# GUOShuxuan/kd-6d-pose-adlp

Measured on AMD Instinct MI355X. Metric: KD train-step images/sec (teacher+student fwd + OT loss + bwd + AdamW), higher is better.
Workload: dtype bf16

## Files before the change

### include/kd6d.h

```cpp
#ifndef KD6D_H
#define KD6D_H

#include <stdint.h>

#ifdef __cplusplus
extern "C" {
#endif

#define KD6D_ABI_VERSION 11

enum { KD6D_BF16 = 0, KD6D_F32 = 1 };
enum { KD6D_ACT_NONE = 0, KD6D_ACT_LEAKY = 1, KD6D_ACT_RELU = 2 };
enum {
  KD6D_OK = 0,
  KD6D_ERR_ARG = -1,
  KD6D_ERR_LAUNCH = -2,
  KD6D_ERR_UNSUPPORTED = -3
};

#define KD6D_MAX_SEG 5

typedef struct kd6d_seg {
  int32_t in_h, in_w;
  int32_t out_h, out_w;
// ... 60 lines not shown
  const kd6d_acc* sums;
  int32_t replicas;
  int32_t act;
  float eps;
  float momentum;
  const float* gamma;
  const float* beta;
  float* running_mean;
  float* running_var;
  float* save_mean;
  float* save_invstd;
} kd6d_bn_in;
int kd6d_conv2d_fwd_block(const kd6d_conv_geom* g, int dtype, const void* x, const kd6d_bn_in* bn, void* z_out,
                          const void* w, float* y_raw, kd6d_acc* stats, int stats_replicas, void* stream);

int kd6d_conv2d_dgrad(const kd6d_conv_geom* g, int dtype, const void* dy,
                      const void* wt, void* dx, int accumulate, void* stream);

int kd6d_conv2d_wgrad_parts(const kd6d_conv_geom* g, int dtype, int with_bias, int cu_budget);
int kd6d_conv2d_wgrad(const kd6d_conv_geom* g, int dtype, const void* x, const void* dy, float* dw_slab,
                      int64_t slab_floats, int64_t* dbias_acc, int64_t acc_hi_stride, int cu_budget, void* stream);

typedef struct kd6d_wgrad_item {
  kd6d_conv_geom geom;
  const void* x;
  const void* dy;
  float* dw;
  float* dbias;
} kd6d_wgrad_item;
int kd6d_wgrad_group_supported(const kd6d_conv_geom* g, int dtype);
int64_t kd6d_wgrad_group_plan(const kd6d_wgrad_item* items, int n_items, int dtype, int n_workgroups, void* plan_host,
                              int64_t plan_capacity, int32_t* info);
int kd6d_wgrad_group_launch(const void* plan_dev, int n_workgroups, int n_reduce_blocks, float* slab_dev, void* stream);

int kd6d_pack_dgrad_weights(int dtype, const void* w_base, void* wt_base,
                            const int32_t* desc_dev, int n_layers,
                            int total_blocks, void* stream);


typedef struct kd6d_levels {
  int32_t n;
  int32_t batch;
  int32_t h[KD6D_MAX_SEG];
  int32_t w[KD6D_MAX_SEG];
  float anchor_stride[KD6D_MAX_SEG];
  float anchor_size[KD6D_MAX_SEG];
} kd6d_levels;

#define KD6D_MAX_GT 4

int kd6d_device_cu_count(void);

typedef struct kd6d_ctx kd6d_ctx;
int kd6d_ctx_create(kd6d_ctx** out);
int kd6d_ctx_destroy(kd6d_ctx* ctx);
int kd6d_ctx_make_current(kd6d_ctx* ctx);
kd6d_ctx* kd6d_ctx_current(void);
int kd6d_ctx_set_option(kd6d_ctx* ctx, const char* name, long long value);
int kd6d_ctx_get_option(kd6d_ctx* ctx, const char* name, long long* value);
int kd6d_ctx_reset_options(kd6d_ctx* ctx);
int kd6d_ctx_barrier_timeouts(kd6d_ctx* ctx);
int kd6d_ctx_conv2d_pair_begin(kd6d_ctx* ctx);
int kd6d_ctx_conv2d_pair_end(kd6d_ctx* ctx);
int kd6d_ctx_conv2d_pair_pending(kd6d_ctx* ctx);

int kd6d_set_option(const char* name, long long value);
// ... 246 lines not shown
```

### kd-6d-pose-adlp_amd/build.py

```python
import hashlib
import os
import subprocess
import sys
from concurrent.futures import ThreadPoolExecutor

HERE = os.path.dirname(os.path.abspath(__file__))
CSRC = os.path.join(HERE, "csrc")
OUT = os.path.join(CSRC, "libkd6d.so")
HIPCC = os.environ.get("HIPCC", "/opt/rocm/bin/hipcc")
FLAGS = [
    "--offload-arch=gfx950", "-O3", "-fPIC", "-std=c++17", "-munsafe-fp-atomics",
    "-Wall", "-Wno-unused-function", "-Wno-unused-variable",
]


EXTRA_FLAGS = {"sinkhorn_dense.hip": ["-mllvm", "-amdgpu-mfma-vgpr-form"],
               "losses.hip": ["-Xclang", "-target-feature", "-Xclang", "-packed-fp32-ops"],
               "sinkhorn.hip": ["-Xclang", "-target-feature", "-Xclang", "-packed-fp32-ops"],
               "augment.hip": ["-Xclang", "-target-feature", "-Xclang", "-packed-fp32-ops"],
               "pnp.hip": ["-Xclang", "-target-feature", "-Xclang", "-packed-fp32-ops"],
               "pose_err.hip": ["-Xclang", "-target-feature", "-Xclang", "-packed-fp32-ops"],
               "bop_err.hip": ["-Xclang", "-target-feature", "-Xclang", "-packed-fp32-ops"],
               "bop_vsd.hip": ["-Xclang", "-target-feature", "-Xclang", "-packed-fp32-ops"],
               "render_frames.hip": ["-Xclang", "-target-feature", "-Xclang", "-packed-fp32-ops"]}


def _sources():
    return sorted(f for f in os.listdir(CSRC) if f.endswith(".hip"))


def _headers_digest():
    h = hashlib.sha256()
    for path in sorted([os.path.join(CSRC, n) for n in os.listdir(CSRC) if n.endswith(".h")]
                       + [os.path.join(HERE, "..", "include", "kd6d.h")]):
        with open(path, "rb") as f:
            h.update(os.path.basename(path).encode())
            h.update(f.read())
    h.update(" ".join(FLAGS).encode())
    return h


def _source_digest(src, base):
    h = base.copy()
    with open(os.path.join(CSRC, src), "rb") as f:
        h.update(f.read())
    h.update(" ".join(EXTRA_FLAGS.get(src, [])).encode())
    return h.hexdigest()


def _san_flags():
    import importlib.util
    path = os.path.join(HERE, "..", "tools", "build_sanitized.py")
    spec = importlib.util.spec_from_file_location("kd6d_build_sanitized", path)
    mod = importlib.util.module_from_spec(spec)
    spec.loader.exec_module(mod)
    return list(mod.SAN_FLAGS)

# ... 64 lines not shown
```

### kd-6d-pose-adlp_amd/csrc/kd6d_common.h

```cpp
#pragma once
#include <hip/hip_runtime.h>
#include <stdint.h>
#include <stdio.h>
#include <string.h>

#include "../../include/kd6d.h"

typedef __bf16 bf16_t;
typedef __bf16 bf16x8_t __attribute__((ext_vector_type(8)));
typedef __bf16 bf16x4_t __attribute__((ext_vector_type(4)));
typedef float f32x4_t __attribute__((ext_vector_type(4)));
typedef float f32x2_t __attribute__((ext_vector_type(2)));
typedef unsigned int u32x4_t __attribute__((ext_vector_type(4)));
typedef unsigned int u32x2_t __attribute__((ext_vector_type(2)));

void kd6d_set_error(const char* fmt, ...);

#define KD6D_CHECK_ARG(cond, ...)              \
  do {                                         \
    if (!(cond)) {                             \
      kd6d_set_error(__VA_ARGS__);             \
      return KD6D_ERR_ARG;                     \
    }                                          \
  } while (0)

#define KD6D_CHECK_LAUNCH(name)                                          \
  do {                                                                   \
    hipError_t e__ = hipGetLastError();                                  \
    if (e__ != hipSuccess) {                                             \
      kd6d_set_error("%s: launch failed: %s", name, hipGetErrorString(e__)); \
      return KD6D_ERR_LAUNCH;                                            \
    }                                                                    \
  } while (0)

enum Kd6dOption {
  KD6D_OPT_CONV_HALO = 0,
  KD6D_OPT_CONV_SMALLC,
  KD6D_OPT_CONV_SPLITK,
  KD6D_OPT_CONV_TILE,
  KD6D_OPT_WGRAD_SMALL,
  KD6D_OPT_BN_ONEPASS,
  KD6D_OPT_BN_ONEPASS_MAX,
  KD6D_OPT_GN_ONEPASS,
  KD6D_OPT_SINKHORN_LANES,
  KD6D_OPT_CONV_HALO_PAIRING,
  KD6D_OPT_CONV_FUSE_NORM,
  KD6D_OPT_SINKHORN_DENSE_MFMA,
  KD6D_OPT_CONV_HALO_WIDE,
  KD6D_OPT_CONV_SMALLC_WMAX,
  KD6D_OPT_SINKHORN_DENSE_SCREEN,
  KD6D_OPT_SINKHORN_DENSE_ROWS,
  KD6D_OPT_STEM_FUSED,
  KD6D_OPT_COUNT
};
long long kd6d_opt(int id);

struct kd6d_ctx {
  long long opt[KD6D_OPT_COUNT];
  void* pair;
  void (*pair_free)(void*);
  unsigned int* timeouts;
  bool owns_timeouts;
};
kd6d_ctx* kd6d_current_ctx();
unsigned int* kd6d_ctx_timeouts_ptr();

template <typename T> __device__ __forceinline__ float to_f32(T v);
template <> __device__ __forceinline__ float to_f32<float>(float v) { return v; }
template <> __device__ __forceinline__ float to_f32<bf16_t>(bf16_t v) { return (float)v; }

template <typename T> __device__ __forceinline__ T from_f32(float v);
template <> __device__ __forceinline__ float from_f32<float>(float v) { return v; }
template <> __device__ __forceinline__ bf16_t from_f32<bf16_t>(float v) { return (bf16_t)v; }

template <auto Kern>
static inline void kd6d_raise_lds_limit(size_t lds) {
  static size_t limit = 0;
  if (lds > limit) {
    (void)hipFuncSetAttribute(reinterpret_cast<const void*>(Kern), hipFuncAttributeMaxDynamicSharedMemorySize, (int)lds);
    limit = lds;
  }
}

template <typename T> struct Granule;
template <> struct Granule<bf16_t> { static constexpr int N = 8; };
// ... 54 lines not shown
```

### kd-6d-pose-adlp_amd/csrc/kd6d_core.hip

```cpp
#include <stdarg.h>

#include "kd6d_common.h"

namespace {
thread_local char g_err[512] = "";
}

void kd6d_set_error(const char* fmt, ...) {
  va_list ap;
  va_start(ap, fmt);
  vsnprintf(g_err, sizeof(g_err), fmt, ap);
  va_end(ap);
}

extern "C" const char* kd6d_last_error(void) { return g_err; }
extern "C" int kd6d_abi_version(void) { return KD6D_ABI_VERSION; }

namespace {
struct OptRow { const char* name; long long def; };
const OptRow kOptRows[KD6D_OPT_COUNT] = {
    {"conv.halo", -1},  {"conv.smallc", -1},       {"conv.splitk", -1}, {"conv.tile", -1},     {"wgrad.small", -1},
    {"bn.onepass", 1},  {"bn.onepass_max", 65536}, {"gn.onepass", 1},   {"sinkhorn.lanes", 1},
    {"conv.halo_pairing", 1}, {"conv.fuse_norm", 3}, {"sinkhorn.dense_mfma", 1}, {"conv.halo_wide", 1},
    {"conv.smallc_wmax", 640}, {"sinkhorn.dense_screen", 1}, {"sinkhorn.dense_rows", -1},
    {"stem.fused", 1},
};
int opt_index(const char* name) {
  if (!name) return -1;
  for (int i = 0; i < KD6D_OPT_COUNT; ++i)
    if (strcmp(name, kOptRows[i].name) == 0) return i;
  return -1;
}

void ctx_defaults(kd6d_ctx* c) {
  for (int i = 0; i < KD6D_OPT_COUNT; ++i) c->opt[i] = kOptRows[i].def;
  c->pair = nullptr; c->pair_free = nullptr; c->timeouts = nullptr; c->owns_timeouts = false;
}

kd6d_ctx* default_ctx() {
  static kd6d_ctx ctx = []() { kd6d_ctx c; ctx_defaults(&c); return c; }();
  return &ctx;
}
thread_local kd6d_ctx* g_current = nullptr;
}

namespace kd6d_detail { unsigned int* barrier_timeouts_device_ptr(); }

kd6d_ctx* kd6d_current_ctx() { return g_current ? g_current : default_ctx(); }

unsigned int* kd6d_ctx_timeouts_ptr() {
  kd6d_ctx* c = kd6d_current_ctx();
  if (!c->timeouts) c->timeouts = kd6d_detail::barrier_timeouts_device_ptr();
  return c->timeouts;
}

long long kd6d_opt(int id) { return kd6d_current_ctx()->opt[id]; }

extern "C" int kd6d_ctx_create(kd6d_ctx** out) {
// ... 168 lines not shown
```

### kd-6d-pose-adlp_amd/kd6d/_lib.py

```python
import ctypes
import os

_HERE = os.path.dirname(os.path.abspath(__file__))
LIB_PATH = os.path.join(os.path.dirname(_HERE), "csrc", "libkd6d.so")

KD6D_BF16 = 0
KD6D_F32 = 1
ACT_NONE, ACT_LEAKY, ACT_RELU = 0, 1, 2
GN_STATS_READY, GN_WS_ZEROED = 1, 2
MAX_SEG = 5
ABI_VERSION = 11
ACC_ACT, ACC_GRAD = 32, 52
NORM_GROUP, NORM_BATCH = 1, 2
BN_FUSED_REPLICAS = 8
NORM_MAX_CTILES = 8


class Seg(ctypes.Structure):
    _fields_ = [("in_h", ctypes.c_int32), ("in_w", ctypes.c_int32),
                ("out_h", ctypes.c_int32), ("out_w", ctypes.c_int32),
                ("in_row0", ctypes.c_int32), ("out_row0", ctypes.c_int32)]


class ConvGeom(ctypes.Structure):
# ... 54 lines not shown
SIGNATURES = {
    "kd6d_abi_version": [],
    "kd6d_device_cu_count": [],
    "kd6d_mark": [_P, _P],
    "kd6d_set_option": [ctypes.c_char_p, ctypes.c_longlong],
    "kd6d_get_option": [ctypes.c_char_p, ctypes.POINTER(ctypes.c_longlong)],
    "kd6d_reset_options": [],
    "kd6d_ctx_create": [ctypes.POINTER(_P)],
    "kd6d_ctx_destroy": [_P],
    "kd6d_ctx_current": [],
    "kd6d_ctx_make_current": [_P],
    "kd6d_ctx_set_option": [_P, ctypes.c_char_p, ctypes.c_longlong],
    "kd6d_ctx_get_option": [_P, ctypes.c_char_p, ctypes.POINTER(ctypes.c_longlong)],
    "kd6d_ctx_reset_options": [_P],
    "kd6d_ctx_barrier_timeouts": [_P],
    "kd6d_ctx_conv2d_pair_begin": [_P],
    "kd6d_ctx_conv2d_pair_end": [_P],
    "kd6d_ctx_conv2d_pair_pending": [_P],
    "kd6d_zero_regions": [ctypes.POINTER(ZeroList), _P, _I, _P],
    "kd6d_uniform_keys": [_P, _I64, _P, ctypes.c_uint64, _P],
    "kd6d_conv2d_fwd": [_G, _I, _P, _P, _P, _P, _P, _I, _P, _P, _I, _P, _I, _P, _I64, _P],
    "kd6d_conv2d_fwd_block": [_G, _I, _P, ctypes.POINTER(BnIn), _P, _P, _P, _P, _I, _P],
    "kd6d_conv2d_fwd_norm_fusable": [_G, _I, _I, _I],
    "kd6d_conv2d_fwd_norm": [_G, _I, _P, _P, _P, _P, ctypes.POINTER(ConvNorm), _P],
    "kd6d_conv2d_dgrad": [_G, _I, _P, _P, _P, _I, _P],
    "kd6d_conv2d_wgrad": [_G, _I, _P, _P, _P, _I64, _P, _I64, _I, _P],
    "kd6d_conv2d_wgrad_parts": [_G, _I, _I, _I],
    "kd6d_acc_read": [_P, _I64, _I, _P, _I, _I, _P],
    "kd6d_grad_acc_resolve": [_P, _I, _I, _P, _I64, _P, _P],
    "kd6d_grad_acc_resolve_part_groups": [_I],
    "kd6d_wgrad_group_supported": [_G, _I],
    "kd6d_wgrad_group_plan": [ctypes.POINTER(WgradItem), _I, _I, _I, _P, _I64, ctypes.POINTER(ctypes.c_int32)],
    "kd6d_wgrad_group_launch": [_P, _I, _I, _P, _P],
    "kd6d_pack_dgrad_weights": [_I, _P, _P, _P, _I, _I, _P],
    "kd6d_colstats": [_I, _P, _I64, _I, _P, _P, _P],
    "kd6d_bn_train_fwd": [_I, _I, _P, _P, _I64, _I, _P, _P, _P, _P, _F, _F, _P, _P, _P, _P, _I, _P],
    "kd6d_bn_train_fwd_res": [_I, _I, _P, _P, _P, _I64, _I, _P, _P, _P, _P, _F, _F, _P, _P, _P, _P, _I, _P],
    "kd6d_bn_train_bwd_reduce": [_I, _I, _P, _P, _I64, _I, _P, _P, _P, _P, _I, _P, _P, _I, _P],
    "kd6d_bn_train_bwd_apply": [_I, _I, _P, _P, _P, _I64, _I, _P, _P, _P, _P, _I, _P, _P, _P, _P, _I, _P],
    "kd6d_barrier_timeouts": [],
    "kd6d_conv2d_pair_begin": [],
    "kd6d_conv2d_pair_end": [],
    "kd6d_conv2d_pair_pending": [],
    "kd6d_bn_pool_train_fwd": [_I, _I, _P, _P, _I, _I, _I, _I, _P, _P, _P, _P, _F, _F, _P, _P, _P, _P, _I, _P],
    "kd6d_bn_pool_train_bwd": [_I, _I, _P, _P, _P, _I, _I, _I, _I, _P, _P, _P, _P, _I, _P, _P, _P, _P, _P, _I, _P],
    "kd6d_bn_pool_train_bwd_reduce": [_I, _I, _P, _P, _I, _I, _I, _I, _P, _P, _P, _P, _I, _P, _P, _I, _P],
    "kd6d_bn_pool_bwd_wgrad_parts": [_G, _I, _I],
    "kd6d_bn_pool_bwd_wgrad": [_G, _I, _P, _P, _P, _P, _P, _P, _P, _I, _P, _P, _I, _P, _P, _P, _I64, _I, _P],
    "kd6d_bn_train_bwd": [_I, _I, _P, _P, _P, _I64, _I, _P, _P, _P, _P, _I, _P, _P, _P, _P, _P, _I, _P],
    "kd6d_gn_relu_fwd": [_I, _I, _P, _P, ctypes.POINTER(ctypes.c_int32), _I, _I, _I, _I, _P, _P, _F, _P, _I, _P],
    "kd6d_gn_relu_bwd": [_I, _I, _P, _P, _P, ctypes.POINTER(ctypes.c_int32), _I, _I, _I, _I, _P, _P, _F, _P,
                         _P, _P, _P, _I64, _I, _P],
    "kd6d_gn_relu_bwd_pair": [_I, _I, ctypes.POINTER(GnItem), ctypes.POINTER(GnItem), ctypes.POINTER(ctypes.c_int32),
                              _I, _I, _I, _I, _F, _I64, _I, _P],
    "kd6d_maxpool2_fwd": [_I, _P, _P, _I, _I, _I, _I, _P],
    "kd6d_maxpool2_bwd": [_I, _P, _P, _P, _I, _I, _I, _I, _I, _P],
    "kd6d_upsample2_add": [_I, _P, _P, _P, _I, _I, _I, _I, _P],
    "kd6d_sumpool2": [_I, _P, _P, _I, _I, _I, _I, _I, _P],
    "kd6d_eltwise": [_I, _I, _P, _P, _P, _I64, _P],
    "kd6d_image_to_nhwc": [_I, _P, _P, _I, _I, _I, _I, _I, _P],
    "kd6d_sinkhorn_div_fwd_bwd": [_P, _P, _P, _P, _P, _P, _P, _P, _I, _F, _F, _F, _F, _P, _P, _P, _P, _P, _P],
    "kd6d_sinkhorn_max_points": [],
    "kd6d_sinkhorn_dense_workspace_floats": [_I, _I, _I],
    "kd6d_sinkhorn_dense_diameter": [_P, _P, _I, _I, _I, _P, _P, _P],
    "kd6d_sinkhorn_dense_fwd_bwd": [_P, _P, _P, _P, _I, _I, _I, _F, _F, _F, _F, _D, _P, _I64, _P, _P, _P, _P],
    "kd6d_teacher_select": [_L, _P, _P, _P, _F, _F, _F, _I, _F, _F, _P, _P, _P, _P, _P, _P, _P],
# ... 85 lines not shown
```

### kd-6d-pose-adlp_amd/kd6d/engine.py

```python
import math

import torch

from . import ops
from .ops import ACT_LEAKY, ACT_NONE, ACT_RELU

ANCHOR_SIZES = [32, 64, 128, 256, 512]
ANCHOR_STRIDES = [8, 16, 32, 64, 128]
TINY_CHANNELS = {
    "darknet_tiny": [[16], [32], [16, 128, 16, 128], [32, 256, 32, 256], [64, 512, 64, 512, 128]],
    "darknet_tiny_h": [[8], [16], [8, 64, 8, 64], [16, 128, 16, 128], [32, 256, 32, 256, 64]],
}
BACKBONE_CFG = {
    "darknet53": ([0, 0, 256, 512, 1024], 256),
    "darknet_tiny": ([0, 0, 128, 128], 256),
    "darknet_tiny_h": ([0, 0, 64, 64], 128),
}


def _pad8(c):
    return (c + 7) // 8 * 8


class Entry:
# ... 222 lines not shown
        return self.net.store.slab(self.w, parts)

    def stem_slab(self, g, dtype):
        budget = self.net.wgrad_budget()
        key = (id(g), dtype, "stem", budget, ops.get_option("stem.fused"))
        parts = self._parts.get(key)
        if parts is None:
            parts = self._parts[key] = ops.bn_pool_bwd_wgrad_parts(g, dtype, budget) if self.b is None else 0
        return self.net.store.slab(self.w, parts) if parts else None

    def bwd(self, x, dy, batch, levels, need_dx=True, dx=None, accumulate=False, need_dw=True):
        st = self.net.store
        g = self.geom(batch, levels)
        grp = self.net.wgrad_group if self.net.grouping else None
        if not need_dw:
            pass
        elif grp is not None and x.dtype == torch.bfloat16 and ops.wgrad_group_supported(g, x.dtype):
            grp.add(g, x, dy, st.storage(self.w, "grads"), None if self.b is None else st.storage(self.b, "grads"),
                    flops=self.flops(g))
        elif (side := self.net.next_side_stream()) is None:
            budget = self.net.wgrad_budget()
            ops.conv2d_wgrad(g, x, dy, self.wgrad_slab(g, x.dtype, budget), flops=self.flops(g),
                             dbias=None if self.b is None else st.acc(self.b), acc_stride=st.acc_stride, cu_budget=budget)
        else:
            budget = self.net.wgrad_budget()
            side.wait_stream(torch.cuda.current_stream())
            with torch.cuda.stream(side):
                ops.conv2d_wgrad(g, x, dy, self.wgrad_slab(g, x.dtype, budget), flops=self.flops(g),
                                 dbias=None if self.b is None else st.acc(self.b), acc_stride=st.acc_stride,
                                 cu_budget=budget)
        if not need_dx:
            return None
        return ops.conv2d_dgrad(g, dy, self.weight_t(), dx=dx, accumulate=accumulate, flops=self.flops(g))


class BatchNorm:
    def __init__(self, net, name, c, trainable=True):
        st = net.store
        self.net, self.c = net, c
        self.gamma = st.add(name + ".weight", "vec", (c,), (c,), trainable)
        self.beta = st.add(name + ".bias", "vec", (c,), (c,), trainable)
        self.rm = st.add(name + ".running_mean", "vec", (c,), (c,), False, region="buf")
        self.rv = st.add(name + ".running_var", "vec", (c,), (c,), False, region="buf")
        self.nbt_index = len(net.bns)
        net.bns.append((name, self))
        self.fold = None

    def folded(self):
        if self.fold is None:
            st = self.net.store
            scale = st.storage(self.gamma) * torch.rsqrt(st.storage(self.rv) + 1e-5)
            shift = st.storage(self.beta) - st.storage(self.rm) * scale
            self.fold = (scale.contiguous(), shift.contiguous())
        return self.fold


class ConvBlock:
    FUSE_STATS_MAX_ROWS = 1 << 15

    @staticmethod
    def bwd_replicas(rows):
        return 8 if rows >= (1 << 14) else 1

    def scratch_floats(self, rows):
        c, A, R = self.conv.cout_p, ops.ACC_FLOATS, self.bwd_replicas(rows)
        return (2 * A + 2 + 2 * A * R) * c + ops.BARRIER_WORDS
# ... 541 lines not shown
                        gn.fwd(raws[tname], B, levels_all, out=y)
                    saved[tname].append((xs[tname], raws[tname]))
                    xs[tname] = y
            for tname, tower, final in towers:
                seg = self.store.storage(self.scales) if tname == "pose" else None
                out, _ = final.fwd(xs[tname], B, levels_all, seg_scale=seg, out_f32=True,
                                   out=self.buf("%s.logits" % tname, (r, final.cout_p), torch.float32))
                self.head_ctx[tname] = (saved[tname], xs[tname])
                outs[tname] = out
            return outs["cls"], outs["pose"]
        for tname, tower, final in towers:
            x = head_in
            saved = []
            for li, (conv, gn) in enumerate(tower):
                y = self.buf("%s.act%d" % (tname, li), (r, oc))
                if self.fuse_norm_on() and conv.norm_fusable(B, levels_all, ops.NORM_GROUP, gn.groups):
                    raw = self.buf("%s.raw%d" % (tname, li), (r, oc), torch.float32) if self.training else None
                    gn.fwd_fused(conv, x, B, levels_all, y, raw_out=raw)
                else:
                    raw, _ = conv.fwd(x, B, levels_all, out_f32=True,
                                      out=self.buf("%s.raw%d" % (tname, li), (r, oc), torch.float32),
                                      stats=gn.stats(B, levels_all), stats_groups=gn.groups)
                    gn.fwd(raw, B, levels_all, out=y)
                saved.append((x, raw))
                x = y
                self._cut()
            seg = self.store.storage(self.scales) if tname == "pose" else None
            out, _ = final.fwd(x, B, levels_all, seg_scale=seg, out_f32=True,
                               out=self.buf("%s.logits" % tname, (r, final.cout_p), torch.float32))
            self.head_ctx[tname] = (saved, x)
            outs[tname] = out
        return outs["cls"], outs["pose"]

    def backward(self, dcls, dreg):
        assert self.training
        B, lv_all, r, oc = self.batch, self.levels, self.rows, self.out_channel
        if self.use_wgrad_group and self.dtype == torch.bfloat16 and self.wgrad_group is None:
            self.wgrad_group = ops.WgradGroup(self.wgrad_group_wgs or max(ops.device_cu_count() // 2, 1))
        self.grouping = self.wgrad_group is not None
        d_head_in = self.buf("d_head_in", (r, oc))
        first = True
        towers = (("cls", self.cls_tower, self.cls_logits, dcls), ("pose", self.pose_tower, self.pose_pred, dreg))
        if self.pair_towers:
            dxs = {}
            for tname, tower, final, dlog in towers:
                saved, last = self.head_ctx[tname]
                dxs[tname] = final.bwd(last, dlog, B, lv_all, dx=self.buf("%s.dact" % tname, (r, oc)))
            for li in range(len(self.cls_tower) - 1, -1, -1):
                draws, items = {}, []
                for tname, tower, _, _ in towers:
                    gn = tower[li][1]
                    draws[tname] = self.buf("%s.draw%d" % (tname, li), (r, oc))
                    items.append(gn.bwd_item(self.head_ctx[tname][0][li][1], dxs[tname], B, lv_all, draws[tname]))
                ops.gn_relu_bwd_pair(items, [h * w for (h, w) in lv_all], B, self.cls_tower[li][1].groups,
                                     self.store.acc_stride, flags=ops.GN_WS_ZEROED)
                if li > 0:
                    with ops.conv_pair(enabled=self.pair_towers == 1):
                        for tname, tower, _, _ in towers:
                            conv = tower[li][0]
                            dxs[tname] = conv.bwd(self.head_ctx[tname][0][li][0], draws[tname], B, lv_all,
                                                  dx=self.buf("%s.dact" % tname, (r, oc)))
                else:
                    for k, (tname, tower, _, _) in enumerate(towers):
                        tower[0][0].bwd(self.head_ctx[tname][0][0][0], draws[tname], B, lv_all, dx=d_head_in,
                                        accumulate=k > 0)
            towers = ()
        for tname, tower, final, dlog in towers:
            saved, last = self.head_ctx[tname]
            dx = final.bwd(last, dlog, B, lv_all, dx=self.buf("%s.dact" % tname, (r, oc)))
            for li in range(len(tower) - 1, -1, -1):
                conv, gn = tower[li]
                x_in, raw = saved[li]
                draw = gn.bwd(raw, dx, B, lv_all, self.buf("%s.draw%d" % (tname, li), (r, oc)))
                if li > 0:
                    dx = conv.bwd(x_in, draw, B, lv_all, dx=self.buf("%s.dact" % tname, (r, oc)))
                else:
                    conv.bwd(x_in, draw, B, lv_all, dx=d_head_in, accumulate=not first)
            first = False
        row0 = self.level_row0
        ops.mark("student.bwd.head.end")

        def dslot(li):
            h, w = lv_all[li]
            return d_head_in[row0[li]:row0[li] + B * h * w]

        idxs = sorted(self.inner.keys())
        n_l = len(idxs)
        grouped_out = set()
        if self.wgrad_group is not None:
            for pos in range(n_l):
                i = idxs[pos]
                f, lv, inner = self.fpn_ctx[i]
                conv = self.outc[i]
                g = conv.geom(B, lv)
                if ops.wgrad_group_supported(g, inner.dtype):
                    self.wgrad_group.add(g, inner, dslot(pos), self.store.storage(conv.w, "grads"),
                                         self.store.storage(conv.b, "grads"), flops=conv.flops(g))
                    grouped_out.add(i)
            if self.wgrad_group_flush != "fpn_end":
                self.flush_wgrad_group()
        self.grouping = False
        ftop, lvtop, p6, p6r, h6 = self.p6_ctx
# ... 83 lines not shown
```

### kd-6d-pose-adlp_amd/kd6d/models/model_kd.py

```python
import torch
from torch import nn

from .. import engine, kd_losses, ops
from ..kd_losses import KDLoss, PackedTargets, TeacherKnowledge


class _Shell(nn.Module):
    """Container used only to reproduce the reference's parameter hierarchy."""


def _get_shell(root, dotted):
    m = root
    for part in dotted:
        nxt = m._modules.get(part)
        if nxt is None:
            nxt = _Shell()
            m.add_module(part, nxt)
        m = nxt
    return m


class _StepFn(torch.autograd.Function):
    @staticmethod
    def forward(ctx, anchor, losses, module):
# ... 236 lines not shown
        tgt = targets if isinstance(targets, PackedTargets) else PackedTargets(targets, net.device)
        pre, side = None, net.side_stream
        keys = getattr(self, "_debug_keys", None)
        if side is not None and net.levels is not None and net.batch == B and net.in_hw == tuple(x.shape[-2:]):
            main = torch.cuda.current_stream()
            side.wait_stream(main)
            with torch.cuda.stream(side):
                pre = self.loss_evaluator.assign(net.levels, B, tgt, keys, prezeroed=prezeroed,
                                                 step_counter=self._nbt if prezeroed else None)
        cls, reg = net.forward(x, scratch_zeroed=prezeroed)
        if pre is not None:
            torch.cuda.current_stream().wait_stream(side)
        ops.mark("student.fwd.end")
        if isinstance(pred_t, kd_losses.DeferredTeacher):
            pred_t = pred_t.join()
        teacher = pred_t if isinstance(pred_t, TeacherKnowledge) else None
        if pred_t is not None and teacher is None:
            raise TypeError("pred_t must come from a kd6d teacher forward (TeacherKnowledge)")
        losses = self.loss_evaluator.forward(cls, reg, net.levels, B, tgt, teacher, keys=keys,
                                             seg_scale=st.storage(net.scales), pre=pre)
        ops.mark("student.loss.end")
        if not prezeroed:
            self._nbt += 1
        return losses

    def step_losses(self, images, targets, pred_t, weights):
        if not self.training:
            raise RuntimeError("step_losses() is the training step")
        x = images.tensors if hasattr(images, "tensors") else images
        if x.device != self.net.device:
            raise RuntimeError("images are on %s but the model is on %s" % (x.device, self.net.device))
        pre = self._begin_step(x)
        losses = self._forward_losses(x, targets, pred_t, prezeroed=pre)
        self._run_backward(weights, dreg_zeroed=pre)
        return losses

    def _run_backward(self, weights, dreg_zeroed=False):
        net, st = self.net, self.net.store
        first = _get_shell(self, ["head", "cls_logits"])._parameters["weight"]
        if first.grad is None:
            self._bind_grads()
        rows = net.rows
        dcls = net.buf("dcls", (rows, 16))
        dreg = net.buf("dreg", (rows, self.net.pose_pred.cout_p))
        if not dreg_zeroed:
            dreg.zero_()
        self.loss_evaluator.backward(weights, net.dtype, dcls, dreg, dseg_scale=st.acc(net.scales),
                                     acc_stride=st.acc_stride)
        ops.mark("student.bwd.start")
        from ..libs import distributed as D
        own = not getattr(self, "_defer_allreduce", False)
        split = D.bucket_split(st) if (own and D.exchange_active() and D.EXCHANGE_MODE == "overlap") else None
        if split is not None:
            comm = self._comm_stream = getattr(self, "_comm_stream", None) or torch.cuda.Stream()

            def early():
                for side in [torch.cuda.current_stream()] + list(net.side_streams or ([net.side_stream] if net.side_stream else [])):
                    comm.wait_stream(side)
                with torch.cuda.stream(comm):
                    st.resolve_grads(split, st.n_train)
                    D.exchange_slice(st, split, st.n_train)
            net.grad_hook = early
            net.resolve_hi = split
        try:
            net.backward(dcls, dreg)
        finally:
            if split is not None:
                net.grad_hook = None
                net.resolve_hi = None
        ops.mark("student.bwd.end")
        if split is not None:
            torch.cuda.current_stream().wait_stream(self._comm_stream)
            D.exchange_slice(st, 0, split)
        elif own:
            D.exchange_gradients(st)
```

### kd-6d-pose-adlp_amd/kd6d/ops.py

```python
import ctypes

import torch

from . import _lib
from ._lib import ACT_LEAKY, ACT_NONE, ACT_RELU, GN_STATS_READY, GN_WS_ZEROED, ConvGeom, check, lib


def dt_code(dtype):
    if dtype == torch.bfloat16:
        return _lib.KD6D_BF16
    if dtype == torch.float32:
        return _lib.KD6D_F32
    raise TypeError("kd6d supports bfloat16 and float32 activations, got %s" % dtype)


def granule(dtype):
    return 8 if dtype == torch.bfloat16 else 4


def _ptr(t):
    if t is None:
        return None
    assert t.is_cuda and t.is_contiguous(), "kd6d ops need contiguous device tensors"
    return ctypes.c_void_p(t.data_ptr())
# ... 164 lines not shown
    assert stats is None or (stats.dtype == torch.float32 and stats.numel() >= stats_replicas * 2 * geom.cout * ACC_FLOATS)
    bn = None
    if bn_in is not None:
        assert x.shape == (geom.rows_in, geom.cin) and x.dtype == torch.float32
        assert z_out is None or (z_out.shape == x.shape and z_out.dtype == w.dtype)
        bn = _lib.BnIn()
        bn.replicas, bn.act = int(bn_in["replicas"]), int(bn_in["act"])
        bn.eps, bn.momentum = float(bn_in.get("eps", 1e-5)), float(bn_in.get("momentum", 0.1))
        assert bn_in["sums"].numel() >= bn.replicas * 2 * geom.cin * ACC_FLOATS
        for name in ("sums", "gamma", "beta", "running_mean", "running_var", "save_mean", "save_invstd"):
            t = bn_in.get(name)
            assert t is None or (t.is_cuda and t.is_contiguous() and t.dtype == torch.float32)
            setattr(bn, name, t.data_ptr() if t is not None else None)
    else:
        assert x.shape == (geom.rows_in, geom.cin) and x.dtype == w.dtype and z_out is None
    with _Timed("conv_fwd", flops, geom):
        check(lib.kd6d_conv2d_fwd_block(geom.ref, dt_code(w.dtype), _ptr(x), ctypes.byref(bn) if bn is not None else None,
                                        _ptr(z_out), _ptr(w), _ptr(y_raw), _ptr(stats), int(stats_replicas), _stream()),
              "kd6d_conv2d_fwd_block")
    return y_raw


def conv2d_dgrad(geom, dy, wt, dx=None, accumulate=False, flops=0):
    assert dy.shape == (geom.rows_out, geom.cout), (dy.shape, geom.rows_out, geom.cout)
    assert wt.dtype == dy.dtype and wt.numel() == geom.cout * geom.ksize * geom.ksize * geom.cin
    if dx is None:
        assert not accumulate
        dx = torch.empty((geom.rows_in, geom.cin), dtype=dy.dtype, device=dy.device)
    assert dx.shape == (geom.rows_in, geom.cin) and dx.dtype == dy.dtype
    with _Timed("conv_dgrad", flops, geom):
        check(lib.kd6d_conv2d_dgrad(geom.ref, dt_code(dy.dtype), _ptr(dy), _ptr(wt), _ptr(dx),
                                    int(accumulate), _stream()), "kd6d_conv2d_dgrad")
    return dx


def conv2d_wgrad_parts(geom, dtype, with_bias=False, cu_budget=0):
    n = int(lib.kd6d_conv2d_wgrad_parts(geom.ref, dt_code(dtype), int(with_bias), int(cu_budget)))
    if n < 1:
        check(n, "kd6d_conv2d_wgrad_parts")
    return n


def conv2d_wgrad(geom, x, dy, dw_slab, flops=0, dbias=None, acc_stride=0, cu_budget=0):
    assert x.shape == (geom.rows_in, geom.cin) and dy.shape == (geom.rows_out, geom.cout)
    assert x.dtype == dy.dtype and dw_slab.dtype == torch.float32 and dw_slab.is_contiguous()
    assert dw_slab.numel() % (geom.cout * geom.ksize * geom.ksize * geom.cin) == 0
    with _Timed("conv_wgrad", flops, geom):
        assert dbias is None or (dbias.dtype == torch.int64 and dbias.numel() >= geom.cout and acc_stride > 0)
        check(lib.kd6d_conv2d_wgrad(geom.ref, dt_code(x.dtype), _ptr(x), _ptr(dy), _ptr(dw_slab), dw_slab.numel(),
                                    _ptr(dbias), int(acc_stride), int(cu_budget), _stream()), "kd6d_conv2d_wgrad")
    return dw_slab


def conv2d_wgrad_f32(geom, x, dy, with_bias=False, cu_budget=0):
    nw = geom.cout * geom.ksize * geom.ksize * geom.cin
    parts = conv2d_wgrad_parts(geom, x.dtype, with_bias, cu_budget)
    slab = torch.empty(parts, nw, dtype=torch.float32, device=x.device)
    acc = planar_acc(geom.cout, x.device) if with_bias else None
    conv2d_wgrad(geom, x, dy, slab, dbias=acc[:geom.cout] if with_bias else None, acc_stride=geom.cout,
                 cu_budget=cu_budget)
    dw = slab[0].clone()
    for k in range(1, parts):
        dw += slab[k]
    return dw, (planar_acc_value(acc) if with_bias else None)


# ... 739 lines not shown
```

Baseline: 6505.

## Add row-sparse backward for pose head conv using positive-anchor row lists

Result: no change. 6471 (-0.5%).

```diff
diff --git a/include/kd6d.h b/include/kd6d.h
--- a/include/kd6d.h
+++ b/include/kd6d.h
@@ -116,6 +116,12 @@
 int64_t kd6d_wgrad_group_plan(const kd6d_wgrad_item* items, int n_items, int dtype, int n_workgroups, void* plan_host,
                               int64_t plan_capacity, int32_t* info);
 int kd6d_wgrad_group_launch(const void* plan_dev, int n_workgroups, int n_reduce_blocks, float* slab_dev, void* stream);
+
+int kd6d_conv2d_rowsparse_supported(const kd6d_conv_geom* g, int dtype, int cap);
+int kd6d_conv2d_rowsparse_dgrad(const kd6d_conv_geom* g, int dtype, const void* dy, const void* wt, void* dx,
+                                int accumulate, const int32_t* cnt, const int32_t* row, int cap, void* stream);
+int kd6d_conv2d_rowsparse_wgrad(const kd6d_conv_geom* g, int dtype, const void* x, const void* dy, float* dw,
+                                float* dbias, const int32_t* cnt, const int32_t* row, int cap, void* stream);
 
 int kd6d_pack_dgrad_weights(int dtype, const void* w_base, void* wt_base,
                             const int32_t* desc_dev, int n_layers,
diff --git a/kd-6d-pose-adlp_amd/build.py b/kd-6d-pose-adlp_amd/build.py
--- a/kd-6d-pose-adlp_amd/build.py
+++ b/kd-6d-pose-adlp_amd/build.py
@@ -22,7 +22,8 @@
                "pose_err.hip": ["-Xclang", "-target-feature", "-Xclang", "-packed-fp32-ops"],
                "bop_err.hip": ["-Xclang", "-target-feature", "-Xclang", "-packed-fp32-ops"],
                "bop_vsd.hip": ["-Xclang", "-target-feature", "-Xclang", "-packed-fp32-ops"],
-               "render_frames.hip": ["-Xclang", "-target-feature", "-Xclang", "-packed-fp32-ops"]}
+               "render_frames.hip": ["-Xclang", "-target-feature", "-Xclang", "-packed-fp32-ops"],
+               "conv_rowsparse.hip": ["-Xclang", "-target-feature", "-Xclang", "-packed-fp32-ops"]}
 
 
 def _sources():
diff --git a/kd-6d-pose-adlp_amd/csrc/conv_rowsparse.hip b/kd-6d-pose-adlp_amd/csrc/conv_rowsparse.hip
--- /dev/null
+++ b/kd-6d-pose-adlp_amd/csrc/conv_rowsparse.hip
@@ -0,0 +1,391 @@
+#include "kd6d_common.h"
+
+namespace {
+
+struct RsLevels {
+  int n, batch, rows;
+  int h[KD6D_MAX_SEG], w[KD6D_MAX_SEG], row0[KD6D_MAX_SEG];
+};
+
+constexpr int kDgWaves = 4;
+constexpr int kDgTile = 64;
+constexpr int kWgThreads = 1024;
+constexpr int kWgWaves = kWgThreads / 64;
+constexpr int kWgSlotsPerThread = 4;
+constexpr int kWgMaxSlots = kWgThreads * kWgSlotsPerThread;
+constexpr int kWgBatch = 8;
+constexpr int kCoBlock = 16, kCiTile = 128, kMaxCout = 256;
+
+__device__ __forceinline__ float bf16_lo(unsigned v) { return __uint_as_float(v << 16); }
+__device__ __forceinline__ float bf16_hi(unsigned v) { return __uint_as_float(v & 0xffff0000u); }
+
+__device__ __forceinline__ int level_of(const RsLevels& L, int r) {
+  int l = 0;
+#pragma unroll
+  for (int s = 1; s < KD6D_MAX_SEG; ++s)
+    if (s < L.n && r >= L.row0[s]) l = s;
+  return l;
+}
+__device__ __forceinline__ void level_dims(const RsLevels& L, int l, int& h, int& w, int& row0) {
+  h = L.h[0]; w = L.w[0]; row0 = L.row0[0];
+#pragma unroll
+  for (int s = 1; s < KD6D_MAX_SEG; ++s)
+    if (s == l) { h = L.h[s]; w = L.w[s]; row0 = L.row0[s]; }
+}
+
+typedef __bf16 rs_bf16x8 __attribute__((ext_vector_type(8)));
+
+__global__ __launch_bounds__(kDgWaves * 64) void rowsparse_dgrad_kernel(
+    const RsLevels L, const bf16_t* __restrict__ dy, const bf16_t* __restrict__ wt, bf16_t* __restrict__ dx,
+    const int* __restrict__ cnt, const int* __restrict__ rowlist, int cap, int cin, int cout, int accumulate) {
+  const int lane = threadIdx.x & 63;
+  const int fr = lane & 15, fq = lane >> 4;
+  const int p = blockIdx.x * kDgWaves + __builtin_amdgcn_readfirstlane((int)(threadIdx.x >> 6));
+  if (p >= L.rows) return;
+  int h, w, row0;
+  level_dims(L, level_of(L, p), h, w, row0);
+  const int hw = h * w;
+  const int b = (p - row0) / hw;
+  const int img0 = row0 + b * hw;
+  const int py = (p - img0) / w, px = (p - img0) - py * w;
+  int tq[9];
+#pragma unroll
+  for (int t = 0; t < 9; ++t) tq[t] = -1;
+  bool any = false;
+  const int n = cnt[b];
+  for (int s0 = 0; s0 < cap; s0 += 64) {
+    const int s = s0 + lane;
+    int tap = -1, q = -1;
+    if (s < cap) q = rowlist[(size_t)b * cap + s];
+    if (s < n) {
+      const int c = q - img0;
+      if (c >= 0 && c < hw) {
+        const int qy = c / w, qx = c - qy * w;
+        const int ky = py - qy + 1, kx = px - qx + 1;
+        if (ky >= 0 && ky <= 2 && kx >= 0 && kx <= 2) tap = ky * 3 + kx;
+      }
+    }
+    if (__ballot(tap >= 0) == 0ull) continue;
+    any = true;
+#pragma unroll
+    for (int t = 0; t < 9; ++t) {
+      const unsigned long long m = __ballot(tap == t);
+      if (tq[t] < 0 && m) tq[t] = __builtin_amdgcn_readlane(q, __ffsll((long long)m) - 1);
+    }
+  }
+  if (!any) {
+    if (!accumulate)
+      for (int c = 8 * lane; c < cin; c += 512)
+        *reinterpret_cast<u32x4_t*>(dx + (size_t)p * cin + c) = u32x4_t{0u, 0u, 0u, 0u};
+    return;
+  }
+
+  u32x2_t dv[9];
+#pragma unroll
+  for (int t = 0; t < 9; ++t) {
+    dv[t] = u32x2_t{0u, 0u};
+    if (tq[t] >= 0 && 4 * lane < cout)
+      dv[t] = *reinterpret_cast<const u32x2_t*>(dy + (size_t)tq[t] * cout + 4 * lane);
+  }
+  unsigned bm[9];
+#pragma unroll
+  for (int t = 0; t < 9; ++t) {
+    unsigned long long m = __ballot(((dv[t].x | dv[t].y) & 0x7fff7fffu) != 0u);
+    m |= m >> 1; m |= m >> 2;
+    unsigned bits = 0u;
+#pragma unroll
+    for (int k = 0; k < kMaxCout / kCoBlock; ++k) bits |= (unsigned)((m >> (4 * k)) & 1ull) << k;
+    bm[t] = bits;
+  }
+
+  const int nb = cout / kCoBlock;
+  const int K = 9 * cout;
+  for (int c0 = 0; c0 < cin; c0 += kDgTile) {
+    f32x4_t acc[kDgTile / 16];
+#pragma unroll
+    for (int i = 0; i < kDgTile / 16; ++i) acc[i] = f32x4_t{0.f, 0.f, 0.f, 0.f};
+    int last_j = -1;
+#pragma unroll
+    for (int t = 0; t < 9; ++t) {
+      unsigned m = bm[t];
+      while (m) {
+        const int blk = __ffs((int)m) - 1;
+        m &= m - 1u;
+        const int j = (t * nb + blk) >> 1;
+        if (j == last_j) continue;
+        last_j = j;
+        const int kk = 32 * j + 8 * fq;
+        const int g = 2 * j + (fq >> 1);
+        int q = tq[t], tl = t;
+        if (t + 1 < 9 && g >= (t + 1) * nb) { q = tq[t + 1 < 9 ? t + 1 : t]; tl = t + 1; }
+        if (t > 0 && g < t * nb) { q = tq[t > 0 ? t - 1 : t]; tl = t - 1; }
+        const bool kvalid = kk < K;
+        rs_bf16x8 fb = {0, 0, 0, 0, 0, 0, 0, 0};
+        if (q >= 0 && kvalid)
+          fb = *reinterpret_cast<const rs_bf16x8*>(dy + (size_t)q * cout + (kk - tl * cout));
+        rs_bf16x8 fa[kDgTile / 16];
+#pragma unroll
+        for (int i = 0; i < kDgTile / 16; ++i) {
+          fa[i] = rs_bf16x8{0, 0, 0, 0, 0, 0, 0, 0};
+          if (kvalid) fa[i] = *reinterpret_cast<const rs_bf16x8*>(wt + (size_t)(c0 + 16 * i + fr) * K + kk);
+        }
+#pragma unroll
+        for (int i = 0; i < kDgTile / 16; ++i)
+          acc[i] = __builtin_amdgcn_mfma_f32_16x16x32_bf16(fa[i], fb, acc[i], 0, 0, 0);
+      }
+    }
+    if (fr < kDgTile / 16) {
+      f32x4_t v = acc[0];
+#pragma unroll
+      for (int i = 1; i < kDgTile / 16; ++i)
+        if (fr == i) v = acc[i];
+      u32x2_t* out = reinterpret_cast<u32x2_t*>(dx + (size_t)p * cin + c0 + 16 * fr + 4 * fq);
+      if (accumulate) {
+        const u32x2_t old = *out;
+        v[0] += bf16_lo(old.x); v[1] += bf16_hi(old.x); v[2] += bf16_lo(old.y); v[3] += bf16_hi(old.y);
+      }
+      *out = u32x2_t{pack_bf16x2(v[0], v[1]), pack_bf16x2(v[2], v[3])};
+    }
+  }
+}
+
+__global__ __launch_bounds__(kWgThreads) void rowsparse_wgrad_kernel(
+    const RsLevels L, const bf16_t* __restrict__ x, const bf16_t* __restrict__ dy, float* __restrict__ dw,
+    float* __restrict__ dbias, const int* __restrict__ cnt, const int* __restrict__ rowlist, int cap, int cin,
+    int cout) {
+  __shared__ __attribute__((aligned(16))) int s_buf[2 * kWgMaxSlots];
+  __shared__ int s_wcnt[kWgWaves];
+  __shared__ float s_bias[kWgWaves][kCoBlock];
+  int* s_q = s_buf;
+  int* s_n = s_buf + kWgMaxSlots;
+  const int tid = threadIdx.x, lane = tid & 63;
+  const int wave = __builtin_amdgcn_readfirstlane(tid >> 6);
+  const int cb = blockIdx.x, tap = blockIdx.y, c0 = blockIdx.z * kCiTile;
+  const int ky = tap / 3, kx = tap - ky * 3;
+  const int nslots = L.batch * cap;
+  const bool do_bias = dbias != nullptr && tap == 4 && blockIdx.z == 0;
+
+  int myr[kWgSlotsPerThread], myn[kWgSlotsPerThread];
+#pragma unroll
+  for (int k = 0; k < kWgSlotsPerThread; ++k) {
+    const int i = tid + k * kWgThreads;
+    int r = -1;
+    if (i < nslots) {
+      const int b = i / cap, s = i - b * cap;
+      if (s < cnt[b]) {
+        r = rowlist[i];
+        if (r < 0 || r >= L.rows) r = -1;
+      }
+    }
+    myr[k] = r;
+    s_q[i] = r;
+  }
+  __syncthreads();
+#pragma unroll
+  for (int k = 0; k < kWgSlotsPerThread; ++k) {
+    const int i = tid + k * kWgThreads;
+    int r = myr[k], nb = -1;
+    if (r >= 0) {
+      const int b = i / cap, s = i - b * cap;
+      int h, w, row0;
+      level_dims(L, level_of(L, r), h, w, row0);
+      const int hw = h * w;
+      const int c = r - row0 - b * hw;
+      bool keep = c >= 0 && c < hw;
+      for (int e = 0; keep && e < s; ++e) keep = s_q[b * cap + e] != r;
+      if (keep) {
+        const u32x4_t* d = reinterpret_cast<const u32x4_t*>(dy + (size_t)r * cout + cb * kCoBlock);
+        const u32x4_t d0 = d[0], d1 = d[1];
+        keep = (((d0.x | d0.y | d0.z | d0.w) | (d1.x | d1.y | d1.z | d1.w)) & 0x7fff7fffu) != 0u;
+      }
+      if (keep) {
+        const int y = c / w, xx = c - y * w;
+        const int ny = y + ky - 1, nx = xx + kx - 1;
+        keep = ny >= 0 && ny < h && nx >= 0 && nx < w;
+        nb = r + (ky - 1) * w + (kx - 1);
+      }
+      if (!keep) r = -1;
+    }
+    myr[k] = r; myn[k] = nb;
+  }
+  __syncthreads();
+  int n = 0;
+#pragma unroll
+  for (int k = 0; k < kWgSlotsPerThread; ++k) {
+    if (k * kWgThreads >= nslots) break;
+    const bool valid = myr[k] >= 0;
+    const unsigned long long m = __ballot(valid);
+    if (lane == 0) s_wcnt[wave] = __popcll(m);
+    __syncthreads();
+    int off = n, tot = 0;
+#pragma unroll
+    for (int v = 0; v < kWgWaves; ++v) {
+      const int c = s_wcnt[v];
+      if (v < wave) off += c;
+      tot += c;
+    }
+    if (valid) {
+      const int pos = off + __popcll(m & ((1ull << lane) - 1ull));
+      s_q[pos] = myr[k]; s_n[pos] = myn[k];
+    }
+    n += tot;
+    __syncthreads();
+  }
+  if (n == 0) return;
+
+  const int lo = (int)((long long)n * wave / kWgWaves), hi = (int)((long long)n * (wave + 1) / kWgWaves);
+  float acc[kCoBlock][2];
+#pragma unroll
+  for (int c = 0; c < kCoBlock; ++c) acc[c][0] = acc[c][1] = 0.f;
+  const bf16_t* xl = x + c0 + 2 * lane;
+  const bf16_t* dyb = dy + cb * kCoBlock;
+  for (int i = lo; i < hi; i += kWgBatch) {
+    unsigned xv[kWgBatch];
+    u32x4_t d0[kWgBatch], d1[kWgBatch];
+#pragma unroll
+    for (int j = 0; j < kWgBatch; ++j) {
+      xv[j] = 0u; d0[j] = d1[j] = u32x4_t{0u, 0u, 0u, 0u};
+      if (i + j < hi) {
+        const int q = __builtin_amdgcn_readfirstlane(s_q[i + j]);
+        const int nb = __builtin_amdgcn_readfirstlane(s_n[i + j]);
+        xv[j] = *reinterpret_cast<const unsigned*>(xl + (size_t)nb * cin);
+        const u32x4_t* d = reinterpret_cast<const u32x4_t*>(dyb + (size_t)q * cout);
+        d0[j] = d[0]; d1[j] = d[1];
+      }
+    }
+#pragma unroll
+    for (int j = 0; j < kWgBatch; ++j) {
+      if (i + j >= hi) break;
+      const float x0 = bf16_lo(xv[j]), x1 = bf16_hi(xv[j]);
+      const unsigned dd[8] = {d0[j].x, d0[j].y, d0[j].z, d0[j].w, d1[j].x, d1[j].y, d1[j].z, d1[j].w};
+#pragma unroll
+      for (int c = 0; c < 8; ++c) {
+        const float da = bf16_lo(dd[c]), db = bf16_hi(dd[c]);
+        acc[2 * c][0] = fmaf(da, x0, acc[2 * c][0]);
+        acc[2 * c][1] = fmaf(da, x1, acc[2 * c][1]);
+        acc[2 * c + 1][0] = fmaf(db, x0, acc[2 * c + 1][0]);
+        acc[2 * c + 1][1] = fmaf(db, x1, acc[2 * c + 1][1]);
+      }
+    }
+  }
+  if (do_bias) {
+    float bs = 0.f;
+    if (lane < kCoBlock) {
+#pragma unroll 8
+      for (int i = lo; i < hi; ++i) bs += to_f32<bf16_t>(dyb[(size_t)s_q[i] * cout + lane]);
+      s_bias[wave][lane] = bs;
+    }
+  }
+  __syncthreads();
+
+  float* s_part = reinterpret_cast<float*>(s_buf);
+  constexpr int kTile = kCoBlock * kCiTile;
+  float t0 = 0.f, t1 = 0.f;
+  for (int round = 0; round < kWgWaves / 4; ++round) {
+    if ((wave >> 2) == round) {
+      float* dst = s_part + (wave & 3) * kTile + 2 * lane;
+#pragma unroll
+      for (int c = 0; c < kCoBlock; ++c) *reinterpret_cast<f32x2_t*>(dst + c * kCiTile) = f32x2_t{acc[c][0], acc[c][1]};
+    }
+    __syncthreads();
+#pragma unroll
+    for (int v = 0; v < 4; ++v) {
+      const f32x2_t pv = *reinterpret_cast<const f32x2_t*>(s_part + v * kTile + 2 * tid);
+      t0 += pv.x; t1 += pv.y;
+    }
+    __syncthreads();
+  }
+  {
+    const int c = tid >> 6, ci = c0 + 2 * lane;
+    f32x2_t* out = reinterpret_cast<f32x2_t*>(dw + ((size_t)(cb * kCoBlock + c) * 9 + tap) * cin + ci);
+    f32x2_t o = *out;
+    o.x += t0; o.y += t1;
+    *out = o;
+  }
+  if (do_bias && tid < kCoBlock) {
+    float bs = 0.f;
+#pragma unroll
+    for (int v = 0; v < kWgWaves; ++v) bs += s_bias[v][tid];
+    dbias[cb * kCoBlock + tid] += bs;
+  }
+}
+
+int rowsparse_params(const kd6d_conv_geom* g, int dtype, int cap, const char* who, RsLevels& L, bool quiet) {
+  if (quiet) {
+    if (!g || dtype != KD6D_BF16 || g->nseg < 1 || g->nseg > KD6D_MAX_SEG || g->ksize != 3 || g->stride != 1 ||
+        g->pad != 1 || g->batch < 1 || cap < 1 || g->cin <= 0 || g->cin % kCiTile || g->cout <= 0 ||
+        g->cout % kCoBlock || g->cout > kMaxCout || (long long)g->batch * cap > kWgMaxSlots)
+      return KD6D_ERR_UNSUPPORTED;
+  } else {
+    KD6D_CHECK_ARG(g != nullptr, "%s: null geometry", who);
+    KD6D_CHECK_ARG(g->nseg >= 1 && g->nseg <= KD6D_MAX_SEG && g->batch >= 1 && cap >= 1, "%s: nseg=%d batch=%d cap=%d",
+                   who, g->nseg, g->batch, cap);
+    if (dtype != KD6D_BF16 || g->ksize != 3 || g->stride != 1 || g->pad != 1 || g->cin <= 0 || g->cin % kCiTile ||
+        g->cout <= 0 || g->cout % kCoBlock || g->cout > kMaxCout || (long long)g->batch * cap > kWgMaxSlots) {
+      kd6d_set_error("%s: takes bf16, 3x3 / stride 1 / pad 1, cin %% %d == 0, cout %% %d == 0, cout <= %d, batch * cap "
+                     "<= %d (got dtype %d, k %d, stride %d, pad %d, cin %d, cout %d, batch %d, cap %d)", who, kCiTile,
+                     kCoBlock, kMaxCout, kWgMaxSlots, dtype, g->ksize, g->stride, g->pad, g->cin, g->cout, g->batch, cap);
+      return KD6D_ERR_UNSUPPORTED;
+    }
+  }
+  long long rows = 0;
+  L.n = g->nseg; L.batch = g->batch;
+  for (int s = 0; s < KD6D_MAX_SEG; ++s) { L.h[s] = L.w[s] = 1; L.row0[s] = 0; }
+  for (int s = 0; s < g->nseg; ++s) {
+    const kd6d_seg& q = g->seg[s];
+    const bool ok = q.in_h > 0 && q.in_w > 0 && q.out_h == q.in_h && q.out_w == q.in_w && q.in_row0 == rows &&
+                    q.out_row0 == rows && (long long)q.in_h * q.in_w <= (1 << 24);
+    if (!ok) {
+      if (!quiet) kd6d_set_error("%s: level %d is not a packed stride-1 level (%dx%d -> %dx%d, rows %d / %d)", who, s,
+                                 q.in_h, q.in_w, q.out_h, q.out_w, q.in_row0, q.out_row0);
+      return quiet ? KD6D_ERR_UNSUPPORTED : KD6D_ERR_ARG;
+    }
+    L.h[s] = q.in_h; L.w[s] = q.in_w; L.row0[s] = (int)rows;
+    rows += (long long)g->batch * q.in_h * q.in_w;
+    if (rows >= (1ll << 30)) {
+      if (!quiet) kd6d_set_error("%s: grid too large", who);
+      return quiet ? KD6D_ERR_UNSUPPORTED : KD6D_ERR_ARG;
+    }
+  }
+  L.rows = (int)rows;
+  return KD6D_OK;
+}
+
+}
+
+extern "C" int kd6d_conv2d_rowsparse_supported(const kd6d_conv_geom* g, int dtype, int cap) {
+  const long long opt = kd6d_opt(KD6D_OPT_HEAD_ROWSPARSE_BWD);
+  if (opt == 0) return 0;
+  RsLevels L;
+  if (rowsparse_params(g, dtype, cap, "kd6d_conv2d_rowsparse_supported", L, true) != KD6D_OK) return 0;
+  return opt == 2 ? 2 : 1;
+}
+
+extern "C" int kd6d_conv2d_rowsparse_dgrad(const kd6d_conv_geom* g, int dtype, const void* dy, const void* wt, void* dx,
+                                           int accumulate, const int32_t* cnt, const int32_t* row, int cap,
+                                           void* stream) {
+  RsLevels L;
+  int rc = rowsparse_params(g, dtype, cap, "kd6d_conv2d_rowsparse_dgrad", L, false);
+  if (rc) return rc;
+  KD6D_CHECK_ARG(dy && wt && dx && cnt && row, "kd6d_conv2d_rowsparse_dgrad: null tensor pointer");
+  hipLaunchKernelGGL(rowsparse_dgrad_kernel, dim3((unsigned)cdiv(L.rows, kDgWaves)), dim3(kDgWaves * 64), 0,
+                     reinterpret_cast<hipStream_t>(stream), L, reinterpret_cast<const bf16_t*>(dy),
+                     reinterpret_cast<const bf16_t*>(wt), reinterpret_cast<bf16_t*>(dx), cnt, row, cap, g->cin, g->cout,
+                     accumulate ? 1 : 0);
+  KD6D_CHECK_LAUNCH("kd6d_conv2d_rowsparse_dgrad");
+  return KD6D_OK;
+}
+
+extern "C" int kd6d_conv2d_rowsparse_wgrad(const kd6d_conv_geom* g, int dtype, const void* x, const void* dy, float* dw,
+                                           float* dbias, const int32_t* cnt, const int32_t* row, int cap,
+                                           void* stream) {
+  RsLevels L;
+  int rc = rowsparse_params(g, dtype, cap, "kd6d_conv2d_rowsparse_wgrad", L, false);
+  if (rc) return rc;
+  KD6D_CHECK_ARG(x && dy && dw && cnt && row, "kd6d_conv2d_rowsparse_wgrad: null tensor pointer");
+  hipLaunchKernelGGL(rowsparse_wgrad_kernel, dim3((unsigned)(g->cout / kCoBlock), 9u, (unsigned)(g->cin / kCiTile)),
+                     dim3(kWgThreads), 0, reinterpret_cast<hipStream_t>(stream), L, reinterpret_cast<const bf16_t*>(x),
+                     reinterpret_cast<const bf16_t*>(dy), dw, dbias, cnt, row, cap, g->cin, g->cout);
+  KD6D_CHECK_LAUNCH("kd6d_conv2d_rowsparse_wgrad");
+  return KD6D_OK;
+}
diff --git a/kd-6d-pose-adlp_amd/csrc/kd6d_common.h b/kd-6d-pose-adlp_amd/csrc/kd6d_common.h
--- a/kd-6d-pose-adlp_amd/csrc/kd6d_common.h
+++ b/kd-6d-pose-adlp_amd/csrc/kd6d_common.h
@@ -51,6 +51,7 @@
   KD6D_OPT_SINKHORN_DENSE_SCREEN,
   KD6D_OPT_SINKHORN_DENSE_ROWS,
   KD6D_OPT_STEM_FUSED,
+  KD6D_OPT_HEAD_ROWSPARSE_BWD,
   KD6D_OPT_COUNT
 };
 long long kd6d_opt(int id);
diff --git a/kd-6d-pose-adlp_amd/csrc/kd6d_core.hip b/kd-6d-pose-adlp_amd/csrc/kd6d_core.hip
--- a/kd-6d-pose-adlp_amd/csrc/kd6d_core.hip
+++ b/kd-6d-pose-adlp_amd/csrc/kd6d_core.hip
@@ -23,7 +23,7 @@
     {"bn.onepass", 1},  {"bn.onepass_max", 65536}, {"gn.onepass", 1},   {"sinkhorn.lanes", 1},
     {"conv.halo_pairing", 1}, {"conv.fuse_norm", 3}, {"sinkhorn.dense_mfma", 1}, {"conv.halo_wide", 1},
     {"conv.smallc_wmax", 640}, {"sinkhorn.dense_screen", 1}, {"sinkhorn.dense_rows", -1},
-    {"stem.fused", 1},
+    {"stem.fused", 1},  {"head.rowsparse_bwd", 1},
 };
 int opt_index(const char* name) {
   if (!name) return -1;
diff --git a/kd-6d-pose-adlp_amd/kd6d/_lib.py b/kd-6d-pose-adlp_amd/kd6d/_lib.py
--- a/kd-6d-pose-adlp_amd/kd6d/_lib.py
+++ b/kd-6d-pose-adlp_amd/kd6d/_lib.py
@@ -110,6 +110,9 @@
     "kd6d_wgrad_group_supported": [_G, _I],
     "kd6d_wgrad_group_plan": [ctypes.POINTER(WgradItem), _I, _I, _I, _P, _I64, ctypes.POINTER(ctypes.c_int32)],
     "kd6d_wgrad_group_launch": [_P, _I, _I, _P, _P],
+    "kd6d_conv2d_rowsparse_supported": [_G, _I, _I],
+    "kd6d_conv2d_rowsparse_dgrad": [_G, _I, _P, _P, _P, _I, _P, _P, _I, _P],
+    "kd6d_conv2d_rowsparse_wgrad": [_G, _I, _P, _P, _P, _P, _P, _P, _I, _P],
     "kd6d_pack_dgrad_weights": [_I, _P, _P, _P, _I, _I, _P],
     "kd6d_colstats": [_I, _P, _I64, _I, _P, _P, _P],
     "kd6d_bn_train_fwd": [_I, _I, _P, _P, _I64, _I, _P, _P, _P, _P, _F, _F, _P, _P, _P, _P, _I, _P],
diff --git a/kd-6d-pose-adlp_amd/kd6d/engine.py b/kd-6d-pose-adlp_amd/kd6d/engine.py
--- a/kd-6d-pose-adlp_amd/kd6d/engine.py
+++ b/kd-6d-pose-adlp_amd/kd6d/engine.py
@@ -278,6 +278,24 @@
         if not need_dx:
             return None
         return ops.conv2d_dgrad(g, dy, self.weight_t(), dx=dx, accumulate=accumulate, flops=self.flops(g))
+
+    def rowsparse_mode(self, batch, levels, cap):
+        key = (batch, tuple(levels), cap, self.net.dtype, "rowsparse", ops.get_option("head.rowsparse_bwd"))
+        mode = self._fusable.get(key)
+        if mode is None:
+            mode = self._fusable[key] = ops.conv_rowsparse_supported(self.geom(batch, levels), self.net.dtype, cap)
+        return mode
+
+    def bwd_rowsparse(self, x, dy, batch, levels, pos, dx, mode):
+        st = self.net.store
+        g = self.geom(batch, levels)
+        cnt, row, cap = pos
+        if mode == 2:
+            ops.conv2d_rowsparse_wgrad(g, x, dy, st.storage(self.w, "grads"), cnt, row, cap,
+                                       dbias=None if self.b is None else st.storage(self.b, "grads"), flops=self.flops(g))
+        else:
+            self.bwd(x, dy, batch, levels, need_dx=False)
+        return ops.conv2d_rowsparse_dgrad(g, dy, self.weight_t(), cnt, row, cap, dx=dx, flops=self.flops(g))
 
 
 class BatchNorm:
@@ -885,9 +903,12 @@
             outs[tname] = out
         return outs["cls"], outs["pose"]
 
-    def backward(self, dcls, dreg):
+    def backward(self, dcls, dreg, pos=None):
         assert self.training
         B, lv_all, r, oc = self.batch, self.levels, self.rows, self.out_channel
+        rs_mode = self.pose_pred.rowsparse_mode(B, lv_all, pos[2]) if pos is not None else 0
+        if rs_mode == 0:
+            pos = None
         if self.use_wgrad_group and self.dtype == torch.bfloat16 and self.wgrad_group is None:
             self.wgrad_group = ops.WgradGroup(self.wgrad_group_wgs or max(ops.device_cu_count() // 2, 1))
         self.grouping = self.wgrad_group is not None
@@ -898,7 +919,11 @@
             dxs = {}
             for tname, tower, final, dlog in towers:
                 saved, last = self.head_ctx[tname]
-                dxs[tname] = final.bwd(last, dlog, B, lv_all, dx=self.buf("%s.dact" % tname, (r, oc)))
+                dact = self.buf("%s.dact" % tname, (r, oc))
+                if pos is not None and final is self.pose_pred:
+                    dxs[tname] = final.bwd_rowsparse(last, dlog, B, lv_all, pos, dact, rs_mode)
+                else:
+                    dxs[tname] = final.bwd(last, dlog, B, lv_all, dx=dact)
             for li in range(len(self.cls_tower) - 1, -1, -1):
                 draws, items = {}, []
                 for tname, tower, _, _ in towers:
@@ -920,7 +945,11 @@
             towers = ()
         for tname, tower, final, dlog in towers:
             saved, last = self.head_ctx[tname]
-            dx = final.bwd(last, dlog, B, lv_all, dx=self.buf("%s.dact" % tname, (r, oc)))
+            dact = self.buf("%s.dact" % tname, (r, oc))
+            if pos is not None and final is self.pose_pred:
+                dx = final.bwd_rowsparse(last, dlog, B, lv_all, pos, dact, rs_mode)
+            else:
+                dx = final.bwd(last, dlog, B, lv_all, dx=dact)
             for li in range(len(tower) - 1, -1, -1):
                 conv, gn = tower[li]
                 x_in, raw = saved[li]
diff --git a/kd-6d-pose-adlp_amd/kd6d/models/model_kd.py b/kd-6d-pose-adlp_amd/kd6d/models/model_kd.py
--- a/kd-6d-pose-adlp_amd/kd6d/models/model_kd.py
+++ b/kd-6d-pose-adlp_amd/kd6d/models/model_kd.py
@@ -292,10 +292,10 @@
             raise RuntimeError("images are on %s but the model is on %s" % (x.device, self.net.device))
         pre = self._begin_step(x)
         losses = self._forward_losses(x, targets, pred_t, prezeroed=pre)
-        self._run_backward(weights, dreg_zeroed=pre)
+        self._run_backward(weights, dreg_zeroed=pre, rowsparse=True)
         return losses
 
-    def _run_backward(self, weights, dreg_zeroed=False):
+    def _run_backward(self, weights, dreg_zeroed=False, rowsparse=False):
         net, st = self.net, self.net.store
         first = _get_shell(self, ["head", "cls_logits"])._parameters["weight"]
         if first.grad is None:
@@ -323,7 +323,8 @@
             net.grad_hook = early
             net.resolve_hi = split
         try:
-            net.backward(dcls, dreg)
+            c = self.loss_evaluator.ctx
+            net.backward(dcls, dreg, pos=(c["pos_cnt"], c["pos_row"], self.loss_evaluator.cap) if rowsparse else None)
         finally:
             if split is not None:
                 net.grad_hook = None
diff --git a/kd-6d-pose-adlp_amd/kd6d/ops.py b/kd-6d-pose-adlp_amd/kd6d/ops.py
--- a/kd-6d-pose-adlp_amd/kd6d/ops.py
+++ b/kd-6d-pose-adlp_amd/kd6d/ops.py
@@ -220,6 +220,45 @@
         check(lib.kd6d_conv2d_dgrad(geom.ref, dt_code(dy.dtype), _ptr(dy), _ptr(wt), _ptr(dx),
                                     int(accumulate), _stream()), "kd6d_conv2d_dgrad")
     return dx
+
+
+def conv_rowsparse_supported(geom, dtype, cap):
+    if dtype != torch.bfloat16:
+        return 0
+    return int(lib.kd6d_conv2d_rowsparse_supported(geom.ref, dt_code(dtype), int(cap)))
+
+
+def _rowlist_check(geom, cnt, row, cap):
+    assert cnt.dtype == torch.int32 and row.dtype == torch.int32
+    assert cnt.numel() >= geom.batch and row.numel() >= geom.batch * cap
+    assert cnt.is_contiguous() and row.is_contiguous()
+
+
+def conv2d_rowsparse_dgrad(geom, dy, wt, cnt, row, cap, dx=None, accumulate=False, flops=0):
+    assert dy.shape == (geom.rows_out, geom.cout), (dy.shape, geom.rows_out, geom.cout)
+    assert wt.dtype == dy.dtype and wt.numel() == geom.cout * geom.ksize * geom.ksize * geom.cin
+    assert dy.data_ptr() % 16 == 0 and wt.data_ptr() % 16 == 0 and (dx is None or dx.data_ptr() % 16 == 0)
+    _rowlist_check(geom, cnt, row, cap)
+    if dx is None:
+        assert not accumulate
+        dx = torch.empty((geom.rows_in, geom.cin), dtype=dy.dtype, device=dy.device)
+    assert dx.shape == (geom.rows_in, geom.cin) and dx.dtype == dy.dtype
+    with _Timed("conv_dgrad", flops, geom):
+        check(lib.kd6d_conv2d_rowsparse_dgrad(geom.ref, dt_code(dy.dtype), _ptr(dy), _ptr(wt), _ptr(dx), int(accumulate),
+                                              _ptr(cnt), _ptr(row), int(cap), _stream()), "kd6d_conv2d_rowsparse_dgrad")
+    return dx
+
+
+def conv2d_rowsparse_wgrad(geom, x, dy, dw, cnt, row, cap, dbias=None, flops=0):
+    assert x.shape == (geom.rows_in, geom.cin) and dy.shape == (geom.rows_out, geom.cout) and x.dtype == dy.dtype
+    assert dw.dtype == torch.float32 and dw.numel() == geom.cout * geom.ksize * geom.ksize * geom.cin
+    assert dbias is None or (dbias.dtype == torch.float32 and dbias.numel() >= geom.cout)
+    assert dy.data_ptr() % 16 == 0 and dw.data_ptr() % 8 == 0
+    _rowlist_check(geom, cnt, row, cap)
+    with _Timed("conv_wgrad", flops, geom):
+        check(lib.kd6d_conv2d_rowsparse_wgrad(geom.ref, dt_code(x.dtype), _ptr(x), _ptr(dy), _ptr(dw), _ptr(dbias),
+                                              _ptr(cnt), _ptr(row), int(cap), _stream()), "kd6d_conv2d_rowsparse_wgrad")
+    return dw
 
 
 def conv2d_wgrad_parts(geom, dtype, with_bias=False, cu_budget=0):
```
